# krocki/Eigen-LSTM

Hardware: AMD Instinct MI355X
Metric: chars/sec fwd+BPTT, enwik6 H=512 S=100 B=64, 1/2/4/8 GPU (higher is better)
Workload: dtype f32; 1 GPU; configs[2] (headline): enwik6.txt, hidden=512 seq=100 batch=64, fp32; run as hidden=512 seq=100 batch=64/GPU (global 64), fp32, enwik6-sized synthetic text (1000000 bytes), stride-1 windows from a full window, Adagrad lr=0.01; parallelism=single, engine=default, gemm=native

## Files before the change

### eigen-lstm_amd/csrc/gemm.hip

```cpp
#include <cstdlib>
#include "kernels.h"

namespace lstmk {
namespace {

typedef float f32x16 __attribute__((ext_vector_type(16)));
typedef float f32x4 __attribute__((ext_vector_type(4)));
typedef float f32x2 __attribute__((ext_vector_type(2)));

#ifdef GEMM_CLOCK_STAMPS
__device__ unsigned long long g_gemm_stamps[2 * 4096];
__device__ unsigned long long g_gemm_timeline[512 * 8 * 4];
#endif

template <int V> struct VecOf;
template <> struct VecOf<1> { using T = float; };
template <> struct VecOf<2> { using T = f32x2; };
template <> struct VecOf<4> { using T = f32x4; };

template <bool KFAST, int V> struct Frag {
    static constexpr int NOFF = KFAST ? V : 1;
    float v[4][V];
    __device__ __forceinline__ void load(const float *__restrict__ X, const unsigned (&off)[NOFF], int ld) {
        if constexpr (KFAST) {
// ... 9 lines not shown
                const typename VecOf<V>::T x = *reinterpret_cast<const typename VecOf<V>::T *>(X + (size_t)j * ld + off[0]);
                if constexpr (V == 1) v[j][0] = x;
                else {
#pragma unroll
                    for (int s = 0; s < V; s++) v[j][s] = x[s];
                }
            }
        }
    }
    __device__ __forceinline__ void load_unit(int u, const float *__restrict__ X, const unsigned (&off)[NOFF], int ld) {
        if constexpr (KFAST) {
            const f32x4 x = *reinterpret_cast<const f32x4 *>(X + off[u]);
#pragma unroll
            for (int j = 0; j < 4; j++) v[j][u] = x[j];
        } else {
            const typename VecOf<V>::T x = *reinterpret_cast<const typename VecOf<V>::T *>(X + (size_t)u * ld + off[0]);
            if constexpr (V == 1) v[u][0] = x;
            else {
#pragma unroll
                for (int s = 0; s < V; s++) v[u][s] = x[s];
            }
        }
    }
    __device__ __forceinline__ void load_tail(const float *__restrict__ X, const unsigned (&off)[NOFF], int ld, int kfirst, int K) {
        static_assert(!KFAST, "k-fast operands need K % 8 == 0");
#pragma unroll
        for (int j = 0; j < 4; j++)
#pragma unroll
            for (int s = 0; s < V; s++) v[j][s] = (kfirst + j < K) ? X[(size_t)j * ld + off[0] + s] : 0.0f;
    }
};

template <bool KFAST, int V> struct Rows {
    static constexpr int TILE = 32 * V;
    static constexpr int NOFF = KFAST ? V : 1;
    __device__ static __forceinline__ int row(int r0, int i, int s) { return KFAST ? r0 + 32 * s + i : r0 + V * i + s; }
    __device__ static __forceinline__ void offsets(unsigned (&off)[NOFF], int ld, int r0, int R, int i, int h) {
        if constexpr (KFAST) {
#pragma unroll
            for (int s = 0; s < V; s++) {
                int r = r0 + 32 * s + i;
                r = r < R ? r : R - 1;
                off[s] = (unsigned)r * (unsigned)ld + 4u * h;
            }
        } else {
            int r = r0 + V * i;
            r = r + V <= R ? r : R - V;
            off[0] = 4u * h * (unsigned)ld + (unsigned)r;
        }
    }
    __device__ static __forceinline__ size_t group_stride(int ld) { return KFAST ? (size_t)8 : (size_t)8 * ld; }
};

template <bool AKF, bool BKF, int VA, int VB, int NW, int DEPTH>
__global__ __launch_bounds__(64 * NW) void k_gemm_regs(int M, int Nn, int K, const float *__restrict__ A, int lda,
                                                       const float *__restrict__ Bm, int ldb, float *__restrict__ C, int ldc,
                                                       int tiles_m, int tiles_n, int kchunk, size_t slab_stride) {
    constexpr int TM = 32 * VA, TN = 32 * VB;
    extern __shared__ __attribute__((aligned(16))) float red[];
    const int tid = threadIdx.x, l = tid & 63, w = __builtin_amdgcn_readfirstlane(tid >> 6);
    const int i = l & 31, h = l >> 5;
    const int ntile = tiles_m * tiles_n;
    int lin = blockIdx.x;
    {
        const int q = ntile >> 3, r = ntile & 7, x = lin & 7;
        lin = (x < r ? x * (q + 1) : r * (q + 1) + (x - r) * q) + (lin >> 3);
    }
    int tm, tn;
    if (tiles_n <= tiles_m) {
        tn = lin % tiles_n;
        tm = lin / tiles_n;
    } else {
        tm = lin % tiles_m;
        tn = lin / tiles_m;
    }
    const int m0 = tm * TM, n0 = tn * TN;
    const int kbeg = blockIdx.y * kchunk;
    const int kend = kbeg + kchunk < K ? kbeg + kchunk : K;
    C += (size_t)blockIdx.y * slab_stride;

    const float *pa = A + (AKF ? (size_t)kbeg : (size_t)kbeg * lda);
    const float *pb = Bm + (BKF ? (size_t)kbeg : (size_t)kbeg * ldb);
    unsigned oa[Rows<AKF, VA>::NOFF], ob[Rows<BKF, VB>::NOFF];
    Rows<AKF, VA>::offsets(oa, lda, m0, M, i, h);
    Rows<BKF, VB>::offsets(ob, ldb, n0, Nn, i, h);
    const size_t sa = Rows<AKF, VA>::group_stride(lda), sb = Rows<BKF, VB>::group_stride(ldb);

    f32x16 acc[VA][VB];
#pragma unroll
    for (int a = 0; a < VA; a++)
#pragma unroll
        for (int b = 0; b < VB; b++)
#pragma unroll
            for (int r = 0; r < 16; r++) acc[a][b][r] = 0.0f;

    auto product = [&](const Frag<AKF, VA> &fa, const Frag<BKF, VB> &fb) {
#pragma unroll
        for (int a = 0; a < VA; a++)
#pragma unroll
            for (int b = 0; b < VB; b++) {
#pragma unroll
                for (int j = 0; j < 4; j++)
                    acc[a][b] = __builtin_amdgcn_mfma_f32_32x32x2f32(fb.v[j][b], fa.v[j][a], acc[a][b], 0, 0, 0);
                __builtin_amdgcn_sched_barrier(0);
            }
    };

#ifdef GEMM_CLOCK_STAMPS
    const unsigned long long st_c0 = __builtin_amdgcn_s_memtime(), st_r0 = __builtin_amdgcn_s_memrealtime();
    if (l == 0 && blockIdx.x < 512 && blockIdx.y == 0) g_gemm_timeline[(blockIdx.x * 8 + w) * 4 + 0] = st_r0;
#endif
    const int nfull = (kend - kbeg) >> 3;
    const int mine = (nfull - w + NW - 1) / NW;
    if (nfull > 0) {
        auto group_of = [&](int n) {
            const int g = w + n * NW;
            return (unsigned)(g < nfull ? g : nfull - 1);
        };
        Frag<AKF, VA> fa[DEPTH];
        Frag<BKF, VB> fb[DEPTH];
#pragma unroll
        for (int d = 0; d < DEPTH; d++) {
            const unsigned g = group_of(d);
            fa[d].load(pa + (size_t)(g * (unsigned)sa), oa, lda);
            fb[d].load(pb + (size_t)(g * (unsigned)sb), ob, ldb);
            __builtin_amdgcn_sched_barrier(0);
        }
        for (int it = 0; it < mine; it += DEPTH) {
#pragma unroll
            for (int d = 0; d < DEPTH; d++) {
                if (it + d < mine) product(fa[d], fb[d]);
                const unsigned g = group_of(it + d + DEPTH);
                fa[d].load(pa + (size_t)(g * (unsigned)sa), oa, lda);
                fb[d].load(pb + (size_t)(g * (unsigned)sb), ob, ldb);
                __builtin_amdgcn_sched_barrier(0);
            }
        }
    }
#ifdef GEMM_CLOCK_STAMPS
    if (tid == 0 && blockIdx.y == 0 && blockIdx.x < 4096) {
        g_gemm_stamps[2 * blockIdx.x] = __builtin_amdgcn_s_memtime() - st_c0;
        g_gemm_stamps[2 * blockIdx.x + 1] = __builtin_amdgcn_s_memrealtime() - st_r0;
    }
    if (l == 0 && blockIdx.x < 512 && blockIdx.y == 0) g_gemm_timeline[(blockIdx.x * 8 + w) * 4 + 1] = __builtin_amdgcn_s_memrealtime();
#endif
    if constexpr (!AKF && !BKF) {
        if (((kend - kbeg) & 7) != 0 && w == nfull % NW) {
            Frag<AKF, VA> ta;
            Frag<BKF, VB> tb;
            const int kfirst = kbeg + nfull * 8 + 4 * h;
            ta.load_tail(pa + (size_t)nfull * sa, oa, lda, kfirst, kend);
            tb.load_tail(pb + (size_t)nfull * sb, ob, ldb, kfirst, kend);
            product(ta, tb);
        }
    }

    constexpr int PIECES = VB * 4;
    f32x4 *part = reinterpret_cast<f32x4 *>(red);
#pragma unroll
    for (int c = 0; c < PIECES; c++) {
        if (c % NW != w) {
            const int b = c >> 2, r4 = c & 3;
#pragma unroll
            for (int a = 0; a < VA; a++) {
                f32x4 x;
#pragma unroll
                for (int e = 0; e < 4; e++) x[e] = acc[a][b][4 * r4 + e];
                part[(((size_t)w * PIECES + c) * VA + a) * 64 + l] = x;
            }
        }
    }
    __syncthreads();
#ifdef GEMM_CLOCK_STAMPS
    if (l == 0 && blockIdx.x < 512 && blockIdx.y == 0) g_gemm_timeline[(blockIdx.x * 8 + w) * 4 + 2] = __builtin_amdgcn_s_memrealtime();
#endif
#pragma unroll
    for (int c = 0; c < PIECES; c++) {
        if (c % NW != w) continue;
        const int b = c >> 2, r4 = c & 3;
        f32x4 s[VA];
#pragma unroll
        for (int a = 0; a < VA; a++) {
#pragma unroll
            for (int ww = 0; ww < NW; ww++) {
                f32x4 x;
                if (ww == w) {
#pragma unroll
                    for (int e = 0; e < 4; e++) x[e] = acc[a][b][4 * r4 + e];
                } else
                    x = part[(((size_t)ww * PIECES + c) * VA + a) * 64 + l];
                if (ww == 0) s[a] = x;
                else {
#pragma unroll
                    for (int e = 0; e < 4; e++) s[a][e] += x[e];
                }
            }
        }
#pragma unroll
        for (int e = 0; e < 4; e++) {
            const int nrow = e + 8 * r4 + 4 * h;
            const int n = Rows<BKF, VB>::row(n0, nrow, b);
            if (n >= Nn) continue;
            float *cp = C + (size_t)n * ldc;
            if constexpr (!AKF && VA > 1) {
                const int m = m0 + VA * i;
                if (m + VA <= M) {
                    typename VecOf<VA>::T x;
#pragma unroll
                    for (int a = 0; a < VA; a++) x[a] = s[a][e];
                    *reinterpret_cast<typename VecOf<VA>::T *>(cp + m) = x;
                }
            } else {
#pragma unroll
                for (int a = 0; a < VA; a++) {
                    const int m = Rows<AKF, VA>::row(m0, i, a);
                    if (m < M) cp[m] = s[a][e];
                }
            }
        }
    }
}

template <bool AKF, bool BKF, int VA, int VB, int NW, int DEPTH>
void launch_regs(int M, int Nn, int K, const float *A, int lda, const float *B, int ldb, float *C, int ldc, int splits,
                 int kchunk, size_t slab_stride, hipStream_t st) {
    constexpr int TM = 32 * VA, TN = 32 * VB;
    const int tiles_m = (M + TM - 1) / TM, tiles_n = (Nn + TN - 1) / TN;
    const size_t lds = sizeof(float) * 4 * 64 * (size_t)NW * VB * 4 * VA;
    auto kern = k_gemm_regs<AKF, BKF, VA, VB, NW, DEPTH>;
    static bool attr_done = false;
    if (!attr_done) {
        (void)hipFuncSetAttribute(reinterpret_cast<const void *>(kern), hipFuncAttributeMaxDynamicSharedMemorySize, (int)lds);
        attr_done = true;
    }
    hipLaunchKernelGGL(kern, dim3(tiles_m * tiles_n, splits), dim3(64 * NW), lds, st, M, Nn, K, A, lda, B, ldb, C, ldc, tiles_m,
                       tiles_n, kchunk, slab_stride);
}

}

int gemm_regs_splits(bool akf, bool bkf, int M, int Nn, int K, int n_cus) {
    if (akf || bkf) return 1;
    const int tiles = ((M + 127) / 128) * ((Nn + 63) / 64);
    int splits = 1;
    while (tiles * splits * 2 <= n_cus && K / (splits * 2) >= 256) splits *= 2;
    return splits;
}

int gemm_regs(bool akf, bool bkf, int M, int Nn, int K, const float *A, int lda, const float *B, int ldb, float *C, int ldc,
              int splits, float *slabs, hipStream_t st) {
    if (splits < 1) splits = 1;
    int kchunk = (K + splits - 1) / splits;
    kchunk = (kchunk + 7) / 8 * 8;
    splits = (K + kchunk - 1) / kchunk;
    float *out = splits > 1 ? slabs : C;
    const int ldo = splits > 1 ? M : ldc;
    const size_t stride = splits > 1 ? (size_t)M * Nn : 0;
    static const bool small_ok = !(getenv("LSTM_HIP_GEMM_SMALL_TILES") && atoi(getenv("LSTM_HIP_GEMM_SMALL_TILES")) == 0);
    const bool small = small_ok && ((M + 127) / 128) * ((Nn + 63) / 64) * splits < 128;
    if (!akf && !bkf && small) launch_regs<false, false, 2, 2, 4, 2>(M, Nn, K, A, lda, B, ldb, out, ldo, splits, kchunk, stride, st);
    else if (!akf && !bkf) launch_regs<false, false, 4, 2, 4, 2>(M, Nn, K, A, lda, B, ldb, out, ldo, splits, kchunk, stride, st);
    else if (!akf && bkf && small) launch_regs<false, true, 2, 2, 4, 2>(M, Nn, K, A, lda, B, ldb, out, ldo, splits, kchunk, stride, st);
    else if (!akf && bkf) launch_regs<false, true, 4, 2, 4, 2>(M, Nn, K, A, lda, B, ldb, out, ldo, splits, kchunk, stride, st);
    else if (akf && bkf) launch_regs<true, true, 2, 2, 4, 2>(M, Nn, K, A, lda, B, ldb, out, ldo, splits, kchunk, stride, st);
    else return -1;
    return splits;
}

void gemm(bool TA, bool TB, int M, int Nn, int K, const float *A, int lda, const float *B, int ldb, float *C, int ldc, int splits,
          float *slabs, hipStream_t st) {
    const int used = gemm_regs(TA, !TB, M, Nn, K, A, lda, B, ldb, C, ldc, splits, slabs, st);
    if (used > 1) gemm_fold(slabs, used, M, Nn, C, ldc, st, 0);
}
int gemm_pick_splits(bool TA, bool TB, int M, int Nn, int K, int n_cus) { return gemm_regs_splits(TA, !TB, M, Nn, K, n_cus); }
int gemm_slabs(bool TA, bool TB, int M, int Nn, int K, const float *A, int lda, const float *B, int ldb, float *slabs, int splits,
               hipStream_t st) {
    return gemm_regs(TA, !TB, M, Nn, K, A, lda, B, ldb, slabs, M, splits, slabs, st);
}

}
```

### eigen-lstm_amd/csrc/kernels.h

```cpp
#pragma once
#include <hip/hip_runtime.h>
#include <stdint.h>

namespace lstmk {

struct ParamLayout {
    size_t W, U, b, Why, by, total;
    __host__ __device__ static ParamLayout make(int N, int M) {
        ParamLayout p;
        p.W = 0;
        p.U = p.W + (size_t)4 * N * M;
        p.b = p.U + (size_t)4 * N * N;
        p.Why = p.b + (size_t)4 * N;
        p.by = p.Why + (size_t)M * N;
        p.total = p.by + (size_t)M;
        return p;
    }
};

enum class FwdForm {
    Step,
    Small,
    Persistent,
    Cols8,
// ... 41 lines not shown
    int half_forms() const { return (fwd == FwdForm::TwoHalf ? 1 : 0) | (bwd == BwdForm::Scatter ? 4 : 0); }
};
EnginePlan plan_engine(int N, int B, unsigned flags, int n_cus);

void pack_U(const float *U, float4 *Ufwd, float4 *Ubwd, int N, hipStream_t st, float4 *Ubwd4 = nullptr,
            float4 *Ufwd4 = nullptr, int half_forms = 0);

void fwd_step(const float4 *Ufwd, const float *W, const float *bias, const float *Hprev, const float *Cprev,
              float *Hout, float *Cout, float *Gout, const int32_t *xi_t, int N, int B, bool fast, hipStream_t st);
void bwd_step(const float4 *Ubwd, const float *DGnext , const float *DHy_t, const float *G_t,
              const float *C_t, const float *Cprev, float *dcnext, float *DG_t, int N, int B, hipStream_t st);

size_t persistent_counter_bytes(int S, int B);
void fwd_persistent(const float4 *Ufwd, const float *W, const float *bias, float *H, float *C, float *G,
                    const int32_t *xi, unsigned *cnt, unsigned *abortp, unsigned epoch, int N, int S, int B, bool fast,
                    hipStream_t st);
int fwd_ring_advance(int ring_base, int S);
void fwd_persistent4(const float4 *Ufwd4, const float *W, const float *bias, float *H, float *C, float *G, const int32_t *xi,
                     float *Hx, unsigned *cnt, unsigned *abortp, unsigned epoch, int ring_base, int N, int S, int B, bool fast,
                     int poll_cfg, hipStream_t st, unsigned long long *stamps = nullptr);
void fwd_persistent6(const float4 *Ufwd5, const float *W, const float *bias, float *H, float *C, float *G, const int32_t *xi,
                     float *Hx, unsigned *cnt, unsigned *abortp, unsigned epoch, int ring_base, int N, int S, int B, bool fast,
                     int poll_cfg, int col0, int cols, int gc, bool pin, hipStream_t st, unsigned long long *stamps);
int bwds_ring_advance(int ring_base, int S);
void bwd_scatter(const float4 *Ubwd6, float *DG, const float *Why, const float *dY, const float *G, const float *C, const float *H,
                 const int32_t *xi, float *gpart, float *Qx, unsigned *cnt, unsigned *abortp, unsigned epoch, int ring_base, int N,
                 int S, int B, int cfg, int col0, int cols, int gc, bool pin, hipStream_t st, unsigned long long *stamps);
void bwd_persistent(const float4 *Ubwd, float *DG, const float *DHy, const float *G, const float *C, const float *H,
                    const int32_t *xi, float *gpart, const float *Why, const float *dY, unsigned *cnt, unsigned *abortp,
                    unsigned epoch, int N, int S, int B, int cols, bool spread, hipStream_t st, unsigned long long *stamps = nullptr,
                    unsigned short *DGb = nullptr);
void pack_U_bf16(const float *U, void *Ufwd16, void *Ubwd16, int N, hipStream_t st);
void fwd_persistent_bf16(const void *Ufwd16, const float *W, const float *bias, float *H, unsigned short *Hb, float *C,
                         float *G, const int32_t *xi, unsigned *cnt, unsigned *abortp, unsigned epoch, int N, int S, int B,
                         bool fast, int cols, hipStream_t st);
void pack_U6_bf16(const float *U, void *Ubwd6b, int N, hipStream_t st);
void pack_Ufwd6_bf16(const float *U, void *img, int N, hipStream_t st);
void fwd_halves_bf16(const void *Ufwd6b, const float *W, const float *bias, float *H, unsigned short *Hb, float *C, float *G,
                     const int32_t *xi, void *Hxb, unsigned *cnt, unsigned *abortp, unsigned epoch, int ring_base, int N, int S,
                     int B, int col0, int cols, int gc, bool pin, bool fast, hipStream_t st, unsigned long long *stamps);
int bwd_scatter_bf16_units(int N);
int bwd_scatter_bf16_ring_advance(int base, int S);
void bwd_scatter_bf16(const void *Ubwd6b, float *DG, const float *DHy, const float *G, const float *C, float *Qx, unsigned *cnt,
                      unsigned *abortp, unsigned epoch, int ring_base, int N, int S, int B, int col0, int cols, int gc, bool pin,
                      hipStream_t st, unsigned long long *stamps, unsigned short *DGt_b = nullptr, int Tpad = 0);
void small_fwd(const float *U, const float *W, const float *bias, float *H, float *C, float *G, const int32_t *xi, int N, int S, bool fast,
               hipStream_t st);
void small_bwd(const float4 *Ubwd, const float *Why, const float *dY, const float *G, const float *C, float *DG, int N, int S, hipStream_t st);
size_t bwd_partial_floats(int N);

void gemm(bool TA, bool TB, int M, int Nn, int K, const float *A, int lda, const float *B, int ldb, float *C, int ldc,
          int splits, float *slabs, hipStream_t st);
int gemm_pick_splits(bool TA, bool TB, int M, int Nn, int K, int n_cus);
void gemm_fold(const float *slabs, int splits, int M, int Nn, float *C, int ldc, hipStream_t st, size_t slab_stride = 0);
int gemm_slabs(bool TA, bool TB, int M, int Nn, int K, const float *A, int lda, const float *B, int ldb, float *slabs, int splits,
               hipStream_t st);
int gemm_regs_splits(bool a_kfast, bool b_kfast, int M, int Nn, int K, int n_cus);
int gemm_regs(bool a_kfast, bool b_kfast, int M, int Nn, int K, const float *A, int lda, const float *B, int ldb, float *C, int ldc,
              int splits, float *slabs, hipStream_t st);

void gemm_bf16(int M, int Nn, int K, const unsigned short *A, int lda, const unsigned short *B, int ldb, float *C, int ldc,
               int splits, float *slabs, hipStream_t st);
int gemm_bf16_pick_splits(int M, int Nn, int K);
void transpose_pack_bf16(const float *src, int K, int R, int ld, unsigned short *dst, int Kpad, hipStream_t st);
void pack_bf16(const float *src, size_t n, unsigned short *dst, hipStream_t st);

int softmax_parts(int T);
void softmax_loss_dy(float *Y, float *P, const float *by, const int32_t *ti, float *colloss, float *dby_part, int col0,
                     int col1, bool stable, hipStream_t st);
void loss_reduce(const float *colloss, int steps, int B, int B_global, double *out, const float *dby_part, int n_parts,
                 float *dby, hipStream_t st, float scale = 1.0f);

constexpr int DW_CHUNK = 32;
size_t dW_scratch_bytes(int T, int G4);
void dW_db(const float *DG , const int32_t *xi , int T, int G4, float *dW , float *db,
           void *scratch, hipStream_t st);
void dW_sort(const int32_t *xi, int T, int G4, void *scratch, hipStream_t st);
void dW_sums(const float *DG, int T, int G4, float *dW, float *db, void *scratch, hipStream_t st);

struct SlideJob {
    const uint8_t *text;
    uint64_t len;
    const uint64_t *pos;
    int32_t *Xr, *Tr;
    const int32_t *headp;
    int32_t *xi, *ti;
    float *H, *C;
    int S, B, N, stride, carry_col;
    uint64_t *pos_out;
    int32_t *head_out;
};
struct TailJob {
    const float *colloss;
    int steps, B, B_global;
    float scale;
    double *loss_out;
    const float *dby_part;
    int n_parts;
};
struct AdamScalars {
    float decay;
    float omb1;
    float b2, omb2;
    float step;
    float bc2s;
    float eps;
// ... 162 lines not shown
```

### eigen-lstm_amd/csrc/lstm_hip_api.cpp

```cpp
#include "../../include/lstm_hip.h"
#include "kernels.h"

#include <dlfcn.h>
#include <hip/hip_runtime.h>

#include <algorithm>
#include <cfloat>
#include <cmath>
#include <cstdarg>
#include <cstdio>
#include <cstring>
#include <map>
#include <mutex>
#include <tuple>
#include <string>
#include <vector>

using namespace lstmk;

namespace {

thread_local char g_err[512] = "";
int fail(int code, const char *fmt, ...) {
    va_list ap;
// ... 63 lines not shown

}

struct lstm_hip_ctx {
    lstm_hip_config cfg{};
    int N_log = 0;
    float *stage = nullptr;
    bool padded() const { return N_log != cfg.N; }
    ParamLayout pl{};
    int T = 0;
    hipStream_t st = nullptr;
    hipStream_t st2 = nullptr;
    hipEvent_t ev0 = nullptr, ev1 = nullptr, ev_fork = nullptr, ev_join = nullptr, ev_mid = nullptr, evt0 = nullptr, evt1 = nullptr;
    bool fold_pending = false;
    int n_slabs_dU = 0;
    bool in_loop = false;
    size_t dU_reduced = 0;
    bool early_reduced = false;
    float *slabs_dU = nullptr;
    EnginePlan plan;
    bool packed16 = false;
    unsigned short *Hb = nullptr, *DGb = nullptr;
    void *Ufwd16 = nullptr, *Ubwd16 = nullptr;
    void *Ubwd6b = nullptr;
    void *Ufwd6b = nullptr;
    unsigned short *Hxb = nullptr;
    bool carry_slide = false, pre_slid = false;
    bool tail = false;
    double *tail_loss = nullptr;
    bool keep_outputs = true;
    bool pr_stale = false, dp_stale = false;
    bool dgt_written = false;
    bool packed6b = false;
    bool packedf6b = false;
    unsigned short *WhyT_b = nullptr, *Why_b = nullptr, *Ht_b = nullptr, *dYt_b = nullptr, *DGt_b = nullptr, *dYb = nullptr;
    int Tpad = 0, SBpad = 0;
    bool why_packed = false;
    float *gpart = nullptr;

    float *P = nullptr, *dP = nullptr, *mem = nullptr;
    float4 *Ufwd = nullptr, *Ubwd = nullptr;
    float4 *Ubwd4 = nullptr;
    float4 *Ufwd4 = nullptr;
    float *Hx = nullptr;
    int ring_base = 0;
    float *DGx = nullptr;
    int ring_base_b = 0;
    bool packed = false;
    float *H = nullptr, *C = nullptr, *G = nullptr, *DG = nullptr, *Y = nullptr, *Pr = nullptr, *DHy = nullptr;
    float *dcnext = nullptr, *colloss = nullptr, *dby_part = nullptr, *slabs = nullptr;
    char *dw_scratch = nullptr;
    int n_dby_parts = 0;
    int splits_dWhy = 1, splits_dU = 1;
    int32_t *xi = nullptr, *ti = nullptr;
    int32_t *Xr = nullptr, *Tr = nullptr, *head = nullptr;
    double *d_loss = nullptr;
    double *d_losses = nullptr;
    double *h_losses = nullptr;
    int64_t losses_cap = 0;
    double clip_max = 0.0;
    double *d_norms = nullptr;
    double *norm_part = nullptr;
    float *clip_coef = nullptr;
    int64_t norms_cap = 0;
    int64_t norms_n = -1;
    int opt_kind = LSTM_HIP_OPT_ADAGRAD;
    double beta1 = 0.0, beta2 = 0.0, adam_eps = 0.0, weight_decay = 0.0;
    int64_t opt_steps = 0;
    float *adam_v = nullptr;
    int avg_kind = LSTM_HIP_AVG_OFF;
    double avg_decay = 0.0;
    int32_t avg_every = 1;
    int64_t avg_seen = 0, avg_n = 0;
    float *avg = nullptr;
    int infer_src = LSTM_HIP_SRC_PARAMS;
    uint8_t *text = nullptr;
    uint64_t text_len = 0;
    uint64_t *pos = nullptr;
    uint64_t *pos_buf = nullptr;
    int32_t *head_buf = nullptr;
    int32_t global_B = 0;
    lstm_hip_ctx *eval_h = nullptr;
    char *gen_scratch = nullptr;
    size_t gen_scratch_bytes = 0;
    int stride = 1, carry_col = 1;
    bool fwd_done = false;
    bool dby_done = false;
    unsigned *cnt = nullptr;
    unsigned *abortp = nullptr;
    size_t cnt_bytes = 0;
    unsigned long long *stamps = nullptr;
    int loss_mode = 0;
    unsigned fwd_epoch = 0, bwd_epoch = 0;
    int64_t counter_resets = 0;

    void *comm = nullptr;
    int nranks = 1, rank = 0;

    bool profiling = false;
    int64_t launches[K_COUNT] = {};
    double total_ms[K_COUNT] = {};
};

namespace {

int launch_status(int id) {
// ... 496 lines not shown
    if (plan.refusal[0]) return fail(LSTM_HIP_EINVAL, "%s", plan.refusal);

    lstm_hip_ctx *h = new lstm_hip_ctx();
    h->N_log = user_cfg->N;
    h->plan = plan;
    const int rc = create_body(h, cfg);
    if (rc != 0) {
        char keep[sizeof(g_err)];
        memcpy(keep, g_err, sizeof(keep));
        (void)lstm_hip_destroy(h);
        memcpy(g_err, keep, sizeof(keep));
        return rc;
    }
    *out = h;
    return 0;
}

}

static int create_body(lstm_hip_ctx *h, const lstm_hip_config *cfg) {
    h->cfg = *cfg;
    h->pl = ParamLayout::make(cfg->N, cfg->M);
    const size_t N = cfg->N, B = cfg->B, S = cfg->S, G4 = 4 * N;
    h->T = (int)((S - 1) * B);
    h->global_B = cfg->B;
    HIP_TRY(hipStreamCreateWithFlags(&h->st, hipStreamNonBlocking));
    HIP_TRY(hipEventCreate(&h->ev0));
    HIP_TRY(hipEventCreate(&h->ev1));
    HIP_TRY(hipEventCreate(&h->evt0));
    HIP_TRY(hipEventCreate(&h->evt1));
    {
        float ms = 0.0f;
        HIP_TRY(hipEventRecord(h->evt0, h->st));
        HIP_TRY(hipEventRecord(h->evt1, h->st));
        HIP_TRY(hipEventSynchronize(h->evt1));
        HIP_TRY(hipEventElapsedTime(&ms, h->evt0, h->evt1));
    }
    const EnginePlan &p = h->plan;
    ALLOC(h->P, h->pl.total);
    ALLOC(h->dP, h->pl.total);
    ALLOC(h->mem, h->pl.total);
    ALLOC(h->H, N * B * S);
    ALLOC(h->C, N * B * S);
    ALLOC(h->G, G4 * B * S);
    ALLOC(h->DG, G4 * B * S);
    ALLOC(h->Y, 256 * B * S);
    ALLOC(h->Pr, 256 * B * S);
    ALLOC(h->DHy, N * B * S);
    ALLOC(h->dcnext, N * B);
    ALLOC(h->colloss, B * S);
    ALLOC(h->dby_part, (size_t)256 * softmax_parts(h->T));
    h->splits_dWhy = gemm_pick_splits(false, true, 256, (int)N, h->T, p.n_cus);
    h->splits_dU = gemm_pick_splits(false, true, (int)G4, (int)N, h->T, p.n_cus);
    if (p.bf16()) {
        h->Tpad = (h->T + 63) / 64 * 64;
        h->SBpad = ((int)B + h->Tpad + 63) / 64 * 64;
        h->splits_dWhy = gemm_bf16_pick_splits(256, (int)N, h->Tpad);
        h->splits_dU = gemm_bf16_pick_splits((int)G4, (int)N, h->Tpad);
    }
    ALLOC(h->slabs, (size_t)h->splits_dWhy * 256 * N);
    ALLOC(h->slabs_dU, (size_t)h->splits_dU * G4 * N);
    ALLOC(h->dw_scratch, dW_scratch_bytes(h->T, (int)G4));
    ALLOC(h->xi, S * B, 0xff);
    ALLOC(h->ti, S * B, 0xff);
    ALLOC(h->Xr, S * B, 0xff);
    ALLOC(h->Tr, S * B, 0xff);
    ALLOC(h->head_buf, 2);
    h->head = h->head_buf;
    ALLOC(h->d_loss, 1);
    ALLOC(h->pos_buf, 2 * (size_t)B);
    h->pos = h->pos_buf;
    h->cnt_bytes = persistent_counter_bytes((int)S, (int)B);
    ALLOC(h->cnt, 2 * h->cnt_bytes / sizeof(unsigned));
    ALLOC(h->abortp, 4);
    if (!p.bf16()) {
        ALLOC(h->Ufwd, N * N);
        ALLOC(h->Ubwd, N * N);
    }
    if (p.ufwd4()) ALLOC(h->Ufwd4, N * N);
    if (p.ubwd4()) ALLOC(h->Ubwd4, N * N);
    if (p.bf16()) {
        ALLOC(h->Hb, S * B * N);
        ALLOC(h->DGb, S * B * G4);
        ALLOC(h->WhyT_b, 256 * N);
        ALLOC(h->Why_b, 256 * N);
        ALLOC(h->Ht_b, N * (size_t)h->SBpad);
        ALLOC(h->dYt_b, (size_t)256 * h->Tpad);
        ALLOC(h->DGt_b, G4 * (size_t)h->Tpad);
        ALLOC(h->dYb, (size_t)h->T * 256);
    }
    if (p.u16) {
        HIP_TRY(hipMalloc(&h->Ufwd16, (size_t)8 * N * N));
        HIP_TRY(hipMalloc(&h->Ubwd16, (size_t)8 * N * N));
    }
    if (p.fwd == FwdForm::Bf16Halves) HIP_TRY(hipMalloc(&h->Ufwd6b, (size_t)8 * N * N));
    if (p.bwd == BwdForm::Bf16Scatter) HIP_TRY(hipMalloc(&h->Ubwd6b, (size_t)8 * N * N));
    if (p.hx_floats) ALLOC(h->Hx, p.hx_floats, 0xff);
    if (p.hxb_halfwords) ALLOC(h->Hxb, p.hxb_halfwords, 0xff);
    if (p.dgx_floats) ALLOC(h->DGx, p.dgx_floats, 0xff);
    if (p.fused) ALLOC(h->gpart, (size_t)((B + p.gpart_cols - 1) / p.gpart_cols) * bwd_partial_floats(cfg->N));
    HIP_TRY(hipStreamCreateWithFlags(&h->st2, hipStreamNonBlocking));
    HIP_TRY(hipEventCreateWithFlags(&h->ev_fork, hipEventDisableTiming));
    HIP_TRY(hipEventCreateWithFlags(&h->ev_join, hipEventDisableTiming));
    HIP_TRY(hipEventCreateWithFlags(&h->ev_mid, hipEventDisableTiming));
    if (p.stamps) ALLOC(h->stamps, 4 * S * 16);
    if (h->padded())
// ... 1481 lines not shown
                     uint64_t *code_off_out, double *bits, uint32_t *trace) {
    CoderRun r;
    if (int rc = coder_begin(h, r, decode, streams, text_off, text_in, code_in, code_off_in, trace != nullptr, 0)) return rc;
    if (int rc = coder_steps(h, r, 0, r.max_len)) return rc;
    return coder_finish(h, r, text_out, code_out, code_off_out, bits, trace, nullptr, 0);
}

int lstm_hip_encode(lstm_hip_t *h, int32_t streams, const uint8_t *text, const uint64_t *text_off, uint8_t *code,
                    uint64_t code_cap, uint64_t *code_off, double *bits, uint32_t *trace) {
    CHECK(h);
    if (streams < 1 || streams > 4096) return fail(LSTM_HIP_EINVAL, "encode: streams must be in [1, 4096] (got %d)", streams);
    if (int rc = check_offsets("encode", "text_off", text_off, streams)) return rc;
    if (!code_off) return fail(LSTM_HIP_EINVAL, "encode: null code_off");
    if (text_off[streams] > 0 && !text) return fail(LSTM_HIP_EINVAL, "encode: null text with %llu bytes to code", (unsigned long long)text_off[streams]);
    uint64_t need = 0;
    for (int s = 0; s < streams; s++) {
        const size_t b = lstm_hip_code_bound(text_off[s + 1] - text_off[s]);
        if (b == SIZE_MAX || need > UINT64_MAX - b) return fail(LSTM_HIP_EINVAL, "encode: text too long");
        need += b;
    }
    if (code_cap < need)
        return fail(LSTM_HIP_EINVAL, "encode: code_cap %llu is below the bound %llu (sum of lstm_hip_code_bound)",
                    (unsigned long long)code_cap, (unsigned long long)need);
    if (need > 0 && !code) return fail(LSTM_HIP_EINVAL, "encode: null code");
    if (h->cfg.N > 16384) return fail(LSTM_HIP_EINVAL, "encode: hidden width %d above 16384", h->cfg.N);
    return run_coder(h, false, streams, text_off, text, nullptr, nullptr, nullptr, code, code_off, bits, trace);
}

int lstm_hip_decode(lstm_hip_t *h, int32_t streams, const uint8_t *code, const uint64_t *code_off, const uint64_t *text_off,
                    uint8_t *text) {
    CHECK(h);
    if (streams < 1 || streams > 4096) return fail(LSTM_HIP_EINVAL, "decode: streams must be in [1, 4096] (got %d)", streams);
    if (int rc = check_offsets("decode", "code_off", code_off, streams)) return rc;
    if (int rc = check_offsets("decode", "text_off", text_off, streams)) return rc;
    if (code_off[streams] > 0 && !code) return fail(LSTM_HIP_EINVAL, "decode: null code with %llu code bytes", (unsigned long long)code_off[streams]);
    if (text_off[streams] > 0 && !text) return fail(LSTM_HIP_EINVAL, "decode: null text with %llu bytes to decode", (unsigned long long)text_off[streams]);
    if (h->cfg.N > 16384) return fail(LSTM_HIP_EINVAL, "decode: hidden width %d above 16384", h->cfg.N);
    return run_coder(h, true, streams, text_off, nullptr, text, code, code_off, nullptr, nullptr, nullptr, nullptr);
}

uint32_t lstm_hip_adaptive_version(void) { return 1; }

int64_t lstm_hip_adaptive_blocks(int32_t S, int32_t B, const uint64_t *text_off) {
    if (S < 2 || B < 1) return fail(LSTM_HIP_EINVAL, "adaptive_blocks: need S >= 2 and B >= 1 (got %d, %d)", S, B);
    if (int rc = check_offsets("adaptive_blocks", "text_off", text_off, B)) return rc;
    uint64_t shortest = UINT64_MAX;
    for (int s = 0; s < B; s++) shortest = std::min<uint64_t>(shortest, text_off[s + 1] - text_off[s]);
    return (int64_t)(shortest / (uint64_t)(S - 1));
}

int lstm_hip_plan_identity(lstm_hip_t *h, char *buf, size_t cap) {
    if (!h || !buf || cap == 0) return fail(LSTM_HIP_EINVAL, "plan_identity: null handle or buffer");
    const EnginePlan &p = h->plan;
    const int n = snprintf(buf, cap, "np%d fwd%d bwd%d fused%d bc%d gp%d fc%d lc%d gc%d quad%d dusplit%d side%d dgt%d sw%d su%d", h->cfg.N,
                           (int)p.fwd, (int)p.bwd, (int)p.fused, p.bwd_cols, p.gpart_cols, p.fwd_cols, p.launch_cols, p.group_cols,
                           (int)p.adagrad_quad, (int)p.du_split, (int)p.side_stream, (int)p.direct_dgt, h->splits_dWhy, h->splits_dU);
    if (n < 0 || (size_t)n >= cap) return fail(LSTM_HIP_EINVAL, "plan_identity: the buffer needs %d bytes", n + 1);
    return 0;
}

static int run_adaptive(lstm_hip_t *h, bool decode, const uint64_t *text_off, const uint8_t *text_in, uint8_t *text_out,
                        const uint8_t *code_in, const uint64_t *code_off_in, uint8_t *code_out, uint64_t *code_off_out, double lr,
                        double *bits, double *block_bits, uint32_t *trace) {
    const int S = h->cfg.S, B = h->cfg.B, N = h->cfg.N;
    const uint64_t L = (uint64_t)(S - 1);
    const int64_t n_blocks = lstm_hip_adaptive_blocks(S, B, text_off);
    if (n_blocks < 0) return (int)n_blocks;
    if (int rc = ensure_losses(h, n_blocks)) return rc;
    h->norms_n = -1;
    h->pre_slid = false;
    const bool clip = h->clip_max > 0.0;
    if (clip)
        if (int rc = ensure_norms(h, n_blocks)) return rc;
    if (int rc = lstm_hip_reset_window(h)) return rc;
    HIP_TRY(hipMemsetAsync(h->H, 0, sizeof(float) * (size_t)S * N * B, h->st));
    HIP_TRY(hipMemsetAsync(h->C, 0, sizeof(float) * (size_t)S * N * B, h->st));
    CoderRun r;
    const int64_t n_bb = decode ? 0 : n_blocks + 1;
    if (int rc = coder_begin(h, r, decode, B, text_off, text_in, code_in, code_off_in, trace != nullptr, n_bb)) return rc;
    BlockWindowArgs w{};
    w.text = r.a.text, w.text_off = r.a.text_off;
    w.xi = h->xi, w.ti = h->ti, w.Xr = h->Xr, w.Tr = h->Tr, w.head = h->head;
    w.H = h->H, w.C = h->C;
    w.bits = r.a.bits, w.bits_prev = r.bits_prev;
    w.S = S, w.B = B, w.NB4 = N * B / 4;
    h->in_loop = true;
    LoopGuard guard{h};
    for (int64_t k = 0; k < n_blocks; k++) {
        int rc = 0;
        if ((rc = coder_steps(h, r, (uint64_t)k * L, (uint64_t)(k + 1) * L))) return rc;
        w.k = k, w.build = 1, w.block_bits = decode ? nullptr : r.block_bits + k;
        RUN(K_BLOCK_WINDOW, block_window(w, h->plan.n_cus, h->st));
        const bool own_loss = loop_window(h, k + 1 == n_blocks, h->d_losses + k);
        if ((rc = do_forward(h))) return rc;
        if (own_loss)
            RUN(K_LOSS, loss_reduce(loss_src(h), loss_steps(h), B, h->global_B, h->d_losses + k, h->dby_part, h->n_dby_parts,
                                    h->dP + h->pl.by, h->st, loss_scale(h)));
        h->dby_done = true;
        if ((rc = do_backward(h))) return rc;
        h->carry_slide = false;
        if ((rc = do_adagrad(h, lr, k))) return rc;
    }
    if (int rc = coder_steps(h, r, (uint64_t)n_blocks * L, r.max_len)) return rc;
    if (!decode) {
        w.k = n_blocks, w.build = 0, w.block_bits = r.block_bits + n_blocks;
        RUN(K_BLOCK_WINDOW, block_window(w, h->plan.n_cus, h->st));
    }
    const int rc = coder_finish(h, r, text_out, code_out, code_off_out, bits, trace, block_bits, n_bb);
    if (int ab = check_abort(h)) return ab;
// ... 94 lines not shown
```

Before: 9.843 million chars/s.

## Chunk GEMM cross-wave reduction through smaller LDS and add opt-in two-blocks-per-CU variant

Folds the per-wave partial accumulators through LDS in rounds of a few pieces instead of all at once, shrinking the dynamic shared memory the register-tiled GEMM needs. Adds a launch_bounds(…,2) kernel variant and a doubled split-K choice for the dU gradient GEMM, enabled only by an environment variable after an occupancy query. The smaller LDS footprint may allow more resident blocks; the chunked fold adds extra barriers. Per-device attribute caching replaces the single static flag.

```diff
diff --git a/eigen-lstm_amd/csrc/gemm.hip b/eigen-lstm_amd/csrc/gemm.hip
--- a/eigen-lstm_amd/csrc/gemm.hip
+++ b/eigen-lstm_amd/csrc/gemm.hip
@@ -85,10 +85,17 @@
     __device__ static __forceinline__ size_t group_stride(int ld) { return KFAST ? (size_t)8 : (size_t)8 * ld; }
 };
 
+template <int VA, int VB, int NW> struct FoldPlan {
+    static constexpr int PIECES = VB * 4;
+    static constexpr int FIT = 64 / (NW * VA);
+    static constexpr int PPP = FIT < 1 ? 1 : (FIT < PIECES ? FIT : PIECES);
+    static constexpr size_t LDS = sizeof(float) * 4 * 64 * (size_t)NW * PPP * VA;
+};
+
 template <bool AKF, bool BKF, int VA, int VB, int NW, int DEPTH>
-__global__ __launch_bounds__(64 * NW) void k_gemm_regs(int M, int Nn, int K, const float *__restrict__ A, int lda,
-                                                       const float *__restrict__ Bm, int ldb, float *__restrict__ C, int ldc,
-                                                       int tiles_m, int tiles_n, int kchunk, size_t slab_stride) {
+__device__ __forceinline__ void gemm_regs_body(int M, int Nn, int K, const float *__restrict__ A, int lda,
+                                               const float *__restrict__ Bm, int ldb, float *__restrict__ C, int ldc,
+                                               int tiles_m, int tiles_n, int kchunk, size_t slab_stride) {
     constexpr int TM = 32 * VA, TN = 32 * VB;
     extern __shared__ __attribute__((aligned(16))) float red[];
     const int tid = threadIdx.x, l = tid & 63, w = __builtin_amdgcn_readfirstlane(tid >> 6);
@@ -188,84 +195,146 @@
         }
     }
 
-    constexpr int PIECES = VB * 4;
+    constexpr int PIECES = VB * 4, PPP = FoldPlan<VA, VB, NW>::PPP;
     f32x4 *part = reinterpret_cast<f32x4 *>(red);
 #pragma unroll
-    for (int c = 0; c < PIECES; c++) {
-        if (c % NW != w) {
+    for (int c0 = 0; c0 < PIECES; c0 += PPP) {
+        if (c0 > 0) __syncthreads();
+#pragma unroll
+        for (int c = c0; c < c0 + PPP && c < PIECES; c++) {
+            if (c % NW != w) {
+                const int b = c >> 2, r4 = c & 3;
+#pragma unroll
+                for (int a = 0; a < VA; a++) {
+                    f32x4 x;
+#pragma unroll
+                    for (int e = 0; e < 4; e++) x[e] = acc[a][b][4 * r4 + e];
+                    part[(((size_t)w * PPP + (c - c0)) * VA + a) * 64 + l] = x;
+                }
+            }
+        }
+        __syncthreads();
+#ifdef GEMM_CLOCK_STAMPS
+        if (c0 + PPP >= PIECES && l == 0 && blockIdx.x < 512 && blockIdx.y == 0)
+            g_gemm_timeline[(blockIdx.x * 8 + w) * 4 + 2] = __builtin_amdgcn_s_memrealtime();
+#endif
+#pragma unroll
+        for (int c = c0; c < c0 + PPP && c < PIECES; c++) {
+            if (c % NW != w) continue;
             const int b = c >> 2, r4 = c & 3;
+            f32x4 s[VA];
 #pragma unroll
             for (int a = 0; a < VA; a++) {
-                f32x4 x;
-#pragma unroll
-                for (int e = 0; e < 4; e++) x[e] = acc[a][b][4 * r4 + e];
-                part[(((size_t)w * PIECES + c) * VA + a) * 64 + l] = x;
-            }
-        }
-    }
-    __syncthreads();
-#ifdef GEMM_CLOCK_STAMPS
-    if (l == 0 && blockIdx.x < 512 && blockIdx.y == 0) g_gemm_timeline[(blockIdx.x * 8 + w) * 4 + 2] = __builtin_amdgcn_s_memrealtime();
-#endif
-#pragma unroll
-    for (int c = 0; c < PIECES; c++) {
-        if (c % NW != w) continue;
-        const int b = c >> 2, r4 = c & 3;
-        f32x4 s[VA];
-#pragma unroll
-        for (int a = 0; a < VA; a++) {
-#pragma unroll
-            for (int ww = 0; ww < NW; ww++) {
-                f32x4 x;
-                if (ww == w) {
-#pragma unroll
-                    for (int e = 0; e < 4; e++) x[e] = acc[a][b][4 * r4 + e];
-                } else
-                    x = part[(((size_t)ww * PIECES + c) * VA + a) * 64 + l];
-                if (ww == 0) s[a] = x;
-                else {
-#pragma unroll
-                    for (int e = 0; e < 4; e++) s[a][e] += x[e];
+#pragma unroll
+                for (int ww = 0; ww < NW; ww++) {
+                    f32x4 x;
+                    if (ww == w) {
+#pragma unroll
+                        for (int e = 0; e < 4; e++) x[e] = acc[a][b][4 * r4 + e];
+                    } else
+                        x = part[(((size_t)ww * PPP + (c - c0)) * VA + a) * 64 + l];
+                    if (ww == 0) s[a] = x;
+                    else {
+#pragma unroll
+                        for (int e = 0; e < 4; e++) s[a][e] += x[e];
+                    }
                 }
             }
-        }
-#pragma unroll
-        for (int e = 0; e < 4; e++) {
-            const int nrow = e + 8 * r4 + 4 * h;
-            const int n = Rows<BKF, VB>::row(n0, nrow, b);
-            if (n >= Nn) continue;
-            float *cp = C + (size_t)n * ldc;
-            if constexpr (!AKF && VA > 1) {
-                const int m = m0 + VA * i;
-                if (m + VA <= M) {
-                    typename VecOf<VA>::T x;
-#pragma unroll
-                    for (int a = 0; a < VA; a++) x[a] = s[a][e];
-                    *reinterpret_cast<typename VecOf<VA>::T *>(cp + m) = x;
+#pragma unroll
+            for (int e = 0; e < 4; e++) {
+                const int nrow = e + 8 * r4 + 4 * h;
+                const int n = Rows<BKF, VB>::row(n0, nrow, b);
+                if (n >= Nn) continue;
+                float *cp = C + (size_t)n * ldc;
+                if constexpr (!AKF && VA > 1) {
+                    const int m = m0 + VA * i;
+                    if (m + VA <= M) {
+                        typename VecOf<VA>::T x;
+#pragma unroll
+                        for (int a = 0; a < VA; a++) x[a] = s[a][e];
+                        *reinterpret_cast<typename VecOf<VA>::T *>(cp + m) = x;
+                    }
+                } else {
+#pragma unroll
+                    for (int a = 0; a < VA; a++) {
+                        const int m = Rows<AKF, VA>::row(m0, i, a);
+                        if (m < M) cp[m] = s[a][e];
+                    }
                 }
-            } else {
-#pragma unroll
-                for (int a = 0; a < VA; a++) {
-                    const int m = Rows<AKF, VA>::row(m0, i, a);
-                    if (m < M) cp[m] = s[a][e];
-                }
             }
         }
     }
 }
 
 template <bool AKF, bool BKF, int VA, int VB, int NW, int DEPTH>
+__global__ __launch_bounds__(64 * NW) void k_gemm_regs(int M, int Nn, int K, const float *__restrict__ A, int lda,
+                                                       const float *__restrict__ Bm, int ldb, float *__restrict__ C, int ldc,
+                                                       int tiles_m, int tiles_n, int kchunk, size_t slab_stride) {
+    gemm_regs_body<AKF, BKF, VA, VB, NW, DEPTH>(M, Nn, K, A, lda, Bm, ldb, C, ldc, tiles_m, tiles_n, kchunk, slab_stride);
+}
+
+template <bool AKF, bool BKF, int VA, int VB, int NW, int DEPTH>
+__global__ __launch_bounds__(64 * NW, 2) void k_gemm_regs_x2(int M, int Nn, int K, const float *__restrict__ A, int lda,
+                                                             const float *__restrict__ Bm, int ldb, float *__restrict__ C,
+                                                             int ldc, int tiles_m, int tiles_n, int kchunk, size_t slab_stride) {
+    gemm_regs_body<AKF, BKF, VA, VB, NW, DEPTH>(M, Nn, K, A, lda, Bm, ldb, C, ldc, tiles_m, tiles_n, kchunk, slab_stride);
+}
+
+constexpr int MAX_DEVICES = 64;
+static int current_device() {
+    int dev = 0;
+    (void)hipGetDevice(&dev);
+    return dev;
+}
+
+static bool per_cu_two_requested() {
+    static const bool two = getenv("LSTM_HIP_GEMM_PER_CU") && atoi(getenv("LSTM_HIP_GEMM_PER_CU")) == 2;
+    return two;
+}
+
+template <bool AKF, bool BKF, int VA, int VB, int NW, int DEPTH> int x2_per_cu() {
+    static signed char known[MAX_DEVICES];
+    if (!per_cu_two_requested()) return 1;
+    const int dev = current_device();
+    if (dev >= 0 && dev < MAX_DEVICES && known[dev]) return known[dev];
+    int nb = 0;
+    auto kern = k_gemm_regs_x2<AKF, BKF, VA, VB, NW, DEPTH>;
+    if (hipOccupancyMaxActiveBlocksPerMultiprocessor(&nb, reinterpret_cast<const void *>(kern), 64 * NW,
+                                                     FoldPlan<VA, VB, NW>::LDS) != hipSuccess) {
+        (void)hipGetLastError();
+        nb = 1;
+    }
+    nb = nb < 1 ? 1 : (nb > 127 ? 127 : nb);
+    if (dev >= 0 && dev < MAX_DEVICES) known[dev] = (signed char)nb;
+    return nb;
+}
+
+template <typename Kern> static void allow_lds(Kern kern, size_t lds, bool (&done)[MAX_DEVICES]) {
+    const int dev = current_device();
+    if (dev >= 0 && dev < MAX_DEVICES && done[dev]) return;
+    (void)hipFuncSetAttribute(reinterpret_cast<const void *>(kern), hipFuncAttributeMaxDynamicSharedMemorySize, (int)lds);
+    if (dev >= 0 && dev < MAX_DEVICES) done[dev] = true;
+}
+
+template <bool AKF, bool BKF, int VA, int VB, int NW, int DEPTH, bool X2 = false>
 void launch_regs(int M, int Nn, int K, const float *A, int lda, const float *B, int ldb, float *C, int ldc, int splits,
                  int kchunk, size_t slab_stride, hipStream_t st) {
     constexpr int TM = 32 * VA, TN = 32 * VB;
     const int tiles_m = (M + TM - 1) / TM, tiles_n = (Nn + TN - 1) / TN;
-    const size_t lds = sizeof(float) * 4 * 64 * (size_t)NW * VB * 4 * VA;
+    const size_t lds = FoldPlan<VA, VB, NW>::LDS;
+    if constexpr (X2) {
+        if (x2_per_cu<AKF, BKF, VA, VB, NW, DEPTH>() >= 2) {
+            auto kern = k_gemm_regs_x2<AKF, BKF, VA, VB, NW, DEPTH>;
+            static bool attr_done[MAX_DEVICES];
+            allow_lds(kern, lds, attr_done);
+            hipLaunchKernelGGL(kern, dim3(tiles_m * tiles_n, splits), dim3(64 * NW), lds, st, M, Nn, K, A, lda, B, ldb, C, ldc,
+                               tiles_m, tiles_n, kchunk, slab_stride);
+            return;
+        }
+    }
     auto kern = k_gemm_regs<AKF, BKF, VA, VB, NW, DEPTH>;
-    static bool attr_done = false;
-    if (!attr_done) {
-        (void)hipFuncSetAttribute(reinterpret_cast<const void *>(kern), hipFuncAttributeMaxDynamicSharedMemorySize, (int)lds);
-        attr_done = true;
-    }
+    static bool attr_done[MAX_DEVICES];
+    allow_lds(kern, lds, attr_done);
     hipLaunchKernelGGL(kern, dim3(tiles_m * tiles_n, splits), dim3(64 * NW), lds, st, M, Nn, K, A, lda, B, ldb, C, ldc, tiles_m,
                        tiles_n, kchunk, slab_stride);
 }
@@ -292,7 +361,7 @@
     static const bool small_ok = !(getenv("LSTM_HIP_GEMM_SMALL_TILES") && atoi(getenv("LSTM_HIP_GEMM_SMALL_TILES")) == 0);
     const bool small = small_ok && ((M + 127) / 128) * ((Nn + 63) / 64) * splits < 128;
     if (!akf && !bkf && small) launch_regs<false, false, 2, 2, 4, 2>(M, Nn, K, A, lda, B, ldb, out, ldo, splits, kchunk, stride, st);
-    else if (!akf && !bkf) launch_regs<false, false, 4, 2, 4, 2>(M, Nn, K, A, lda, B, ldb, out, ldo, splits, kchunk, stride, st);
+    else if (!akf && !bkf) launch_regs<false, false, 4, 2, 4, 2, true>(M, Nn, K, A, lda, B, ldb, out, ldo, splits, kchunk, stride, st);
     else if (!akf && bkf && small) launch_regs<false, true, 2, 2, 4, 2>(M, Nn, K, A, lda, B, ldb, out, ldo, splits, kchunk, stride, st);
     else if (!akf && bkf) launch_regs<false, true, 4, 2, 4, 2>(M, Nn, K, A, lda, B, ldb, out, ldo, splits, kchunk, stride, st);
     else if (akf && bkf) launch_regs<true, true, 2, 2, 4, 2>(M, Nn, K, A, lda, B, ldb, out, ldo, splits, kchunk, stride, st);
@@ -306,6 +375,16 @@
     if (used > 1) gemm_fold(slabs, used, M, Nn, C, ldc, st, 0);
 }
 int gemm_pick_splits(bool TA, bool TB, int M, int Nn, int K, int n_cus) { return gemm_regs_splits(TA, !TB, M, Nn, K, n_cus); }
+int gemm_regs_per_cu() {
+    const int nb = x2_per_cu<false, false, 4, 2, 4, 2>();
+    return nb >= 2 ? 2 : 1;
+}
+int gemm_window_splits(int library_splits, int M, int Nn, int K, int n_cus, int per_cu) {
+    const int tiles = ((M + 127) / 128) * ((Nn + 63) / 64);
+    const bool small = tiles * library_splits < 128;
+    if (per_cu < 2 || small || tiles * library_splits > n_cus || K / (library_splits * 2) < 256) return library_splits;
+    return library_splits * 2;
+}
 int gemm_slabs(bool TA, bool TB, int M, int Nn, int K, const float *A, int lda, const float *B, int ldb, float *slabs, int splits,
                hipStream_t st) {
     return gemm_regs(TA, !TB, M, Nn, K, A, lda, B, ldb, slabs, M, splits, slabs, st);
diff --git a/eigen-lstm_amd/csrc/kernels.h b/eigen-lstm_amd/csrc/kernels.h
--- a/eigen-lstm_amd/csrc/kernels.h
+++ b/eigen-lstm_amd/csrc/kernels.h
@@ -117,6 +117,8 @@
 void gemm(bool TA, bool TB, int M, int Nn, int K, const float *A, int lda, const float *B, int ldb, float *C, int ldc,
           int splits, float *slabs, hipStream_t st);
 int gemm_pick_splits(bool TA, bool TB, int M, int Nn, int K, int n_cus);
+int gemm_regs_per_cu();
+int gemm_window_splits(int library_splits, int M, int Nn, int K, int n_cus, int per_cu);
 void gemm_fold(const float *slabs, int splits, int M, int Nn, float *C, int ldc, hipStream_t st, size_t slab_stride = 0);
 int gemm_slabs(bool TA, bool TB, int M, int Nn, int K, const float *A, int lda, const float *B, int ldb, float *slabs, int splits,
                hipStream_t st);
diff --git a/eigen-lstm_amd/csrc/lstm_hip_api.cpp b/eigen-lstm_amd/csrc/lstm_hip_api.cpp
--- a/eigen-lstm_amd/csrc/lstm_hip_api.cpp
+++ b/eigen-lstm_amd/csrc/lstm_hip_api.cpp
@@ -139,6 +139,7 @@
     char *dw_scratch = nullptr;
     int n_dby_parts = 0;
     int splits_dWhy = 1, splits_dU = 1;
+    int gemm_per_cu = 1;
     int32_t *xi = nullptr, *ti = nullptr;
     int32_t *Xr = nullptr, *Tr = nullptr, *head = nullptr;
     double *d_loss = nullptr;
@@ -741,6 +742,8 @@
     ALLOC(h->dby_part, (size_t)256 * softmax_parts(h->T));
     h->splits_dWhy = gemm_pick_splits(false, true, 256, (int)N, h->T, p.n_cus);
     h->splits_dU = gemm_pick_splits(false, true, (int)G4, (int)N, h->T, p.n_cus);
+    h->gemm_per_cu = gemm_regs_per_cu();
+    h->splits_dU = gemm_window_splits(h->splits_dU, (int)G4, (int)N, h->T, p.n_cus, h->gemm_per_cu);
     if (p.bf16()) {
         h->Tpad = (h->T + 63) / 64 * 64;
         h->SBpad = ((int)B + h->Tpad + 63) / 64 * 64;
@@ -2328,9 +2331,10 @@
 int lstm_hip_plan_identity(lstm_hip_t *h, char *buf, size_t cap) {
     if (!h || !buf || cap == 0) return fail(LSTM_HIP_EINVAL, "plan_identity: null handle or buffer");
     const EnginePlan &p = h->plan;
-    const int n = snprintf(buf, cap, "np%d fwd%d bwd%d fused%d bc%d gp%d fc%d lc%d gc%d quad%d dusplit%d side%d dgt%d sw%d su%d", h->cfg.N,
+    const int n = snprintf(buf, cap, "np%d fwd%d bwd%d fused%d bc%d gp%d fc%d lc%d gc%d quad%d dusplit%d side%d dgt%d sw%d su%d%s", h->cfg.N,
                            (int)p.fwd, (int)p.bwd, (int)p.fused, p.bwd_cols, p.gpart_cols, p.fwd_cols, p.launch_cols, p.group_cols,
-                           (int)p.adagrad_quad, (int)p.du_split, (int)p.side_stream, (int)p.direct_dgt, h->splits_dWhy, h->splits_dU);
+                           (int)p.adagrad_quad, (int)p.du_split, (int)p.side_stream, (int)p.direct_dgt, h->splits_dWhy, h->splits_dU,
+                           h->gemm_per_cu == 2 ? " pcu2" : "");
     if (n < 0 || (size_t)n >= cap) return fail(LSTM_HIP_EINVAL, "plan_identity: the buffer needs %d bytes", n + 1);
     return 0;
 }
```

Result: no change. 9.810 million chars/s (-0.3%).
